# louissmit/VBNN

Hardware: AMD Instinct MI355X
Metric: VBLinear fwd+bwd samples/sec (higher is better)
Workload: dtype bf16; 1 GPU; 784-4096-4096-10 VBLinear MLP, batch 4096 per GPU, LRT, S=1; mode=lrt, global_batch=4096, parallelism=dp1, warmup_steps_run=250, backward_order=every updateGradInput, then the accGradParameters from the first layer up, launch=one stream launch per kernel

## Files before the change

vbnn_amd/csrc/elementwise.hip:

```cpp
#include "common.h"

static inline int grid_for(int64_t work_items, int per_block) {
    int64_t b = (work_items + per_block - 1) / per_block;
    if (b < 1) b = 1;
    if (b > 2048) b = 2048;
    return (int)b;
}

template <bool HW>
__global__ __launch_bounds__(256) void k_fill_normal(float* out, int64_t rows, int64_t cols, int64_t ld, uint64_t seed,
                                                     uint32_t stream, uint32_t layer, uint32_t draw, int64_t row0, float scale) {
    const int64_t quads = (cols + 3) >> 2;
    const int64_t total = rows * quads;
    for (int64_t t = (int64_t)blockIdx.x * 256 + threadIdx.x; t < total; t += (int64_t)gridDim.x * 256) {
        const int64_t r = t / quads, q = t - r * quads;
        const vbnn_f32x4 z = HW ? vbnn_normal4_hw(seed, stream, layer, draw, (uint32_t)(row0 + r), (uint32_t)q)
                                : vbnn_normal4(seed, stream, layer, draw, (uint32_t)(row0 + r), (uint32_t)q);
        float* p = out + r * ld + q * 4;
        const int valid = (int)min((int64_t)4, cols - q * 4);
        const bool vec = ((ld & 3) == 0) && (((uintptr_t)out & 15u) == 0);
        store4<float>(p, z.v[0] * scale, z.v[1] * scale, z.v[2] * scale, z.v[3] * scale, valid, vec);
    }
}

// ... 1289 lines not shown
            const int rr = idx >> 4, c4 = (idx & 15) * 4;
            const int64_t r = r0 + rr, c = c0 + c4;
            float a[4] = {0.f, 0.f, 0.f, 0.f}, b[4] = {0.f, 0.f, 0.f, 0.f};
            const int valid = (r < N) ? (int)min((int64_t)4, I - c) : 0;
            if (valid > 0) {
                load4<float>(src + (rpd > 0 ? r % rpd : r) * ld_src + c, a, valid, vec_in);
#pragma unroll
                for (int e = 0; e < 4; ++e) { const float ar = Elt<T>::from(Elt<T>::to(a[e])); b[e] = ar * ar; }
                store4<T>(x_s + r * ld_x + c, a[0], a[1], a[2], a[3], valid, true);
                if (x2_s) store4<T>(x2_s + r * ld_x + c, b[0], b[1], b[2], b[3], valid, true);
            }
#pragma unroll
            for (int e = 0; e < 4; ++e) { ta[rr][c4 + e] = a[e]; tb[rr][c4 + e] = b[e]; }
        }
        if (xT_s) {
            __syncthreads();
#pragma unroll
            for (int k = 0; k < 4; ++k) {
                const int idx = threadIdx.x + 256 * k;
                const int cc = idx >> 4, r4 = (idx & 15) * 4;
                const int64_t c = c0 + cc, r = r0 + r4;
                const int valid = (c < I) ? (int)min((int64_t)4, N - r) : 0;
                if (valid > 0) {
                    store4<T>(xT_s + c * ld_xT + r, ta[r4][cc], ta[r4 + 1][cc], ta[r4 + 2][cc], ta[r4 + 3][cc], valid, vec_t);
                    if (x2T_s)
                        store4<T>(x2T_s + c * ld_xT + r, tb[r4][cc], tb[r4 + 1][cc], tb[r4 + 2][cc], tb[r4 + 3][cc], valid, vec_t);
                }
            }
            __syncthreads();
        }
    }
}

extern "C" int vbnn_pack_input(vbnn_ctx* ctx, int dtype, const float* src, int64_t ld_src, int64_t N, int64_t I, void* x_s,
                               void* x2_s, int64_t ld_x, void* xT_s, void* x2T_s, int64_t ld_xT, int64_t rows_per_draw) {
    VBNN_API_BEGIN
    VBNN_REQUIRE(ctx && src && x_s, "null argument");
    VBNN_REQUIRE(rows_per_draw >= 0, "rows_per_draw");
    VBNN_REQUIRE(N > 0 && I > 0 && ld_src >= I && ld_x >= I && ld_x % 4 == 0, "shape");
    VBNN_REQUIRE(!x2T_s || xT_s, "x2T_s needs xT_s");
    VBNN_REQUIRE(!xT_s || ld_xT >= N, "ld_xT");
    const int64_t ntiles = ((N + 63) / 64) * ((I + 63) / 64);
    const int nb = (int)(ntiles < 4096 ? ntiles : 4096);
    if (dtype == VBNN_F32)
        hipLaunchKernelGGL(k_pack_input<float>, dim3(nb), dim3(256), 0, ctx->stream, src, ld_src, N, I, (float*)x_s, (float*)x2_s,
                           ld_x, (float*)xT_s, (float*)x2T_s, ld_xT, rows_per_draw);
    else if (dtype == VBNN_BF16)
        hipLaunchKernelGGL(k_pack_input<bf16_t>, dim3(nb), dim3(256), 0, ctx->stream, src, ld_src, N, I, (bf16_t*)x_s,
                           (bf16_t*)x2_s, ld_x, (bf16_t*)xT_s, (bf16_t*)x2T_s, ld_xT, rows_per_draw);
    else { vbnn_set_error("unsupported dtype %d", dtype); return VBNN_ERR_UNSUPPORTED; }
    return vbnn_check_launch("k_pack_input");
    VBNN_API_END
}

template <bool TO_BF16>
__global__ __launch_bounds__(256) void k_cast_grads(const void* __restrict__ src, void* __restrict__ dst, int64_t n, int vec) {
    const int64_t i0 = ((int64_t)blockIdx.x * 256 + threadIdx.x) * 8;
    if (i0 >= n) return;
    if (vec && i0 + 8 <= n) {
        if constexpr (TO_BF16) {
            const f32x4 a = reinterpret_cast<const f32x4*>(static_cast<const float*>(src) + i0)[0];
            const f32x4 b = reinterpret_cast<const f32x4*>(static_cast<const float*>(src) + i0)[1];
            reinterpret_cast<bf16x8*>(static_cast<bf16_t*>(dst) + i0)[0] =
                bf16x8{(bf16_t)a[0], (bf16_t)a[1], (bf16_t)a[2], (bf16_t)a[3], (bf16_t)b[0], (bf16_t)b[1], (bf16_t)b[2], (bf16_t)b[3]};
        } else {
            const bf16x8 v = reinterpret_cast<const bf16x8*>(static_cast<const bf16_t*>(src) + i0)[0];
            reinterpret_cast<f32x4*>(static_cast<float*>(dst) + i0)[0] = f32x4{(float)v[0], (float)v[1], (float)v[2], (float)v[3]};
            reinterpret_cast<f32x4*>(static_cast<float*>(dst) + i0)[1] = f32x4{(float)v[4], (float)v[5], (float)v[6], (float)v[7]};
        }
    } else {
        for (int64_t i = i0; i < n && i < i0 + 8; ++i) {
            if constexpr (TO_BF16) static_cast<bf16_t*>(dst)[i] = (bf16_t)static_cast<const float*>(src)[i];
            else static_cast<float*>(dst)[i] = (float)static_cast<const bf16_t*>(src)[i];
        }
// ... 67 lines not shown
```

vbnn_amd/csrc/head.hip:

```cpp
#include "common.h"
#include "gemm_v1.h"

constexpr int HEAD_CMAX = 16;
constexpr int HEAD_FW = 8;

template <typename T> struct Vec8;
template <> struct Vec8<bf16_t> {
    typedef bf16x8 raw_t;
    static __device__ __forceinline__ raw_t load_raw(const bf16_t* p) { return *reinterpret_cast<const bf16x8*>(p); }
    static __device__ __forceinline__ void cvt(const raw_t& t, float (&v)[8]) {
#pragma unroll
        for (int e = 0; e < 8; ++e) v[e] = (float)t[e];
    }
    static __device__ __forceinline__ raw_t load_guarded(const bf16_t* p, int valid) {
        raw_t t;
#pragma unroll
        for (int e = 0; e < 8; ++e) t[e] = e < valid ? p[e] : (bf16_t)0.f;
        return t;
    }
    static __device__ __forceinline__ void load(const bf16_t* p, float (&v)[8]) {
        const bf16x8 t = *reinterpret_cast<const bf16x8*>(p);
#pragma unroll
        for (int e = 0; e < 8; ++e) v[e] = (float)t[e];
    }
// ... 33 lines not shown
__device__ __forceinline__ float head_sum_partials(const float* src, int64_t stride, int R) {
    float tot = 0.f;
    int r = 0;
    for (; r + 8 <= R; r += 8) {
        float p[8];
#pragma unroll
        for (int u = 0; u < 8; ++u) p[u] = vbnn_load_wt(src + (int64_t)(r + u) * stride);
#pragma unroll
        for (int u = 0; u < 8; ++u) tot += p[u];
    }
    if (r < R) {
        float p[8];
#pragma unroll
        for (int u = 0; u < 8; ++u) p[u] = (r + u < R) ? vbnn_load_wt(src + (int64_t)(r + u) * stride) : 0.f;
#pragma unroll
        for (int u = 0; u < 8; ++u) if (r + u < R) tot += p[u];
    }
    return tot;
}

__device__ __forceinline__ void head_row_max(const float (&v)[4], int q, float& mx, int& arg) {
    mx = -INFINITY; arg = 0x7fffffff;
#pragma unroll
    for (int j = 0; j < 4; ++j)
        if (v[j] > mx) { mx = v[j]; arg = 4 * q + j; }
#pragma unroll
    for (int off = 16; off <= 32; off <<= 1) {
        const float om = __shfl_xor(mx, off, 64);
        const int oa = __shfl_xor(arg, off, 64);
        if (om > mx || (om == mx && oa < arg)) { mx = om; arg = oa; }
    }
}

__device__ __forceinline__ void head_log_softmax(f32x4 s, int q, int C, const float* __restrict__ bias, float (&lg)[4], int& arg, float& lse) {
#pragma unroll
    for (int j = 0; j < 4; ++j) {
        const int c = 4 * q + j;
        lg[j] = (c < C) ? s[j] + (bias ? bias[c] : 0.f) : -INFINITY;
    }
    float mx;
    head_row_max(lg, q, mx, arg);
    float se = 0.f;
#pragma unroll
    for (int j = 0; j < 4; ++j) if (4 * q + j < C) se += expf(lg[j] - mx);
    se += __shfl_xor(se, 16, 64);
    se += __shfl_xor(se, 32, 64);
    lse = mx + logf(se);
}

__device__ __forceinline__ void head_rows_from_logits(f32x4 s, int lane, int64_t n0, int64_t N, int C, const float* __restrict__ bias,
                                                      const int32_t* __restrict__ target, int64_t rpd, float inv_n, float* out, float* g_logits,
                                                      float* logits, double* part_loss, int32_t* part_corr) {
    const int q = lane >> 4, c16 = lane & 15;
    const int64_t n = n0 + c16;
    const bool row_ok = n < N;
    float lg[4];
    int arg;
    float lse;
    head_log_softmax(s, q, C, bias, lg, arg, lse);
    const int t = row_ok ? min(max(target[rpd > 0 ? n % rpd : n], 0), C - 1) : 0;
    double loss_acc = 0.0;
#pragma unroll
    for (int j = 0; j < 4; ++j) {
        const int c = 4 * q + j;
        if (row_ok && c < C) {
            const float o = lg[j] - lse;
            if (logits) logits[n * C + c] = lg[j];
            if (out) out[n * C + c] = o;
            g_logits[n * C + c] = (expf(o) - (c == t ? 1.0f : 0.0f)) * inv_n;
            if (c == t) loss_acc -= (double)o * (double)inv_n;
        }
    }
    int corr = (row_ok && q == 0 && arg == t) ? 1 : 0;
#pragma unroll
    for (int off = 32; off > 0; off >>= 1) { loss_acc += __shfl_xor(loss_acc, off, 64); corr += __shfl_xor(corr, off, 64); }
    if (lane == 0) { vbnn_store_wt(&part_loss[blockIdx.x], loss_acc); vbnn_store_wt(&part_corr[blockIdx.x], (int32_t)corr); }
}

template <int NT>
__device__ __forceinline__ void head_sum_loss_partials(unsigned* counter, const double* part_loss, const int32_t* part_corr, double* loss_sum,
                                                       int32_t* correct, int accumulate, double* red_l, int* red_c, int* last) {
    if (!vbnn_last_arriver(counter, gridDim.x, last)) return;
    const int lane = threadIdx.x & 63, wave = threadIdx.x >> 6;
    double ls = 0.0;
    int cs = 0;
    for (int b = (int)threadIdx.x; b < (int)gridDim.x; b += NT) { ls += vbnn_load_wt(&part_loss[b]); cs += vbnn_load_wt(&part_corr[b]); }
#pragma unroll
    for (int off = 32; off > 0; off >>= 1) { ls += __shfl_xor(ls, off, 64); cs += __shfl_xor(cs, off, 64); }
    if (lane == 0) { red_l[wave] = ls; red_c[wave] = cs; }
    __syncthreads();
    if (threadIdx.x == 0) {
        double lt = 0.0;
        int ct = 0;
#pragma unroll
        for (int w = 0; w < NT / 64; ++w) { lt += red_l[w]; ct += red_c[w]; }
        if (loss_sum) loss_sum[0] = (accumulate ? loss_sum[0] : 0.0) + lt;
        if (correct) correct[0] = (accumulate ? correct[0] : 0) + ct;
    }
}

template <typename T>
__device__ __forceinline__ f32x4 head_logits_wave(const T* __restrict__ hp, const T* __restrict__ wp, int64_t k_lo, int64_t k_hi) {
    constexpr int KE = 64 / (int)sizeof(T);
    typedef typename Frag<T>::type frag_t;
    f32x4 acc = {0.f, 0.f, 0.f, 0.f};
    int64_t ks = k_lo;
    for (; ks + 16 <= k_hi; ks += 16) {
        frag_t a[16], b[16];
#pragma unroll
        for (int u = 0; u < 16; ++u) {
            a[u] = *reinterpret_cast<const frag_t*>(wp + (ks + u) * KE);
            b[u] = *reinterpret_cast<const frag_t*>(hp + (ks + u) * KE);
        }
#pragma unroll
        for (int u = 0; u < 16; ++u) acc = mfma_step<T>(a[u], b[u], acc);
    }
    for (; ks + 8 <= k_hi; ks += 8) {
        frag_t a[8], b[8];
#pragma unroll
// ... 35 lines not shown
    __shared__ int red_c[HEAD_FW];
    __shared__ int last;
    const int lane = threadIdx.x & 63, wave = threadIdx.x >> 6;
    const int64_t n0 = (int64_t)blockIdx.x * 16;
    const int q = lane >> 4, c16 = lane & 15;
    const T* hp = h + min(n0 + c16, N - 1) * ld_h + q * CE;
    const T* wp = w3 + (int64_t)min(c16, C - 1) * ld_w + q * CE;
    const int64_t ksteps = Hp / KE;
    const int64_t k_lo = ksteps * wave / HEAD_FW, k_hi = ksteps * (wave + 1) / HEAD_FW;
    const f32x4 acc = head_logits_wave<T>(hp, wp, k_lo, k_hi);
    part[wave][lane] = acc;
    __syncthreads();
    if (wave == 0) {
        f32x4 s = part[0][lane];
#pragma unroll
        for (int w = 1; w < HEAD_FW; ++w) s += part[w][lane];
        head_rows_from_logits(s, lane, n0, N, C, bias, target, rpd, inv_n, out, g_logits, logits, part_loss, part_corr);
    }
    head_sum_loss_partials<64 * HEAD_FW>(counter, part_loss, part_corr, loss_sum, correct, accumulate, red_l, red_c, &last);
}

__global__ __launch_bounds__(64) void k_head_from_slots(const float* __restrict__ slots, int n_slots, const float* __restrict__ bias,
                                                        const int32_t* __restrict__ target, int64_t N, int C, float inv_n, float* out,
                                                        float* g_logits, float* logits, double* loss_sum, int32_t* correct, int accumulate,
                                                        double* part_loss, int32_t* part_corr, unsigned* counter, int64_t rpd) {
    __shared__ double red_l[1];
    __shared__ int red_c[1];
    __shared__ int last;
    const int lane = threadIdx.x;
    const int64_t n0 = (int64_t)blockIdx.x * 16;
    const int q = lane >> 4, c16 = lane & 15;
    const float* p = slots + (min(n0 + c16, N - 1) * 16 + 4 * q);
    const int64_t stride = N * 16;
    f32x4 s = {0.f, 0.f, 0.f, 0.f};
    int k = 0;
    for (; k + 16 <= n_slots; k += 16) {
        f32x4 v[16];
#pragma unroll
        for (int u = 0; u < 16; ++u) v[u] = *reinterpret_cast<const f32x4*>(p + (int64_t)(k + u) * stride);
#pragma unroll
        for (int u = 0; u < 16; ++u) s += v[u];
    }
    for (; k + 2 <= n_slots; k += 2) {
        f32x4 v[2];
#pragma unroll
        for (int u = 0; u < 2; ++u) v[u] = *reinterpret_cast<const f32x4*>(p + (int64_t)(k + u) * stride);
        s += v[0]; s += v[1];
    }
    for (; k < n_slots; ++k) s += *reinterpret_cast<const f32x4*>(p + (int64_t)k * stride);
    head_rows_from_logits(s, lane, n0, N, C, bias, target, rpd, inv_n, out, g_logits, logits, part_loss, part_corr);
    head_sum_loss_partials<64>(counter, part_loss, part_corr, loss_sum, correct, accumulate, red_l, red_c, &last);
}

__device__ __forceinline__ float head_row_entropy(const float (&o)[4], int q, int C) {
    float e = 0.f;
#pragma unroll
    for (int j = 0; j < 4; ++j) if (4 * q + j < C) e = fmaf(expf(o[j]), o[j], e);
    e += __shfl_xor(e, 16, 64);
    e += __shfl_xor(e, 32, 64);
    return -e;
}

__device__ __forceinline__ float head_logaddexp(float a, float b) {
    const float m = fmaxf(a, b);
    return m + log1pf(expf(fminf(a, b) - m));
}

template <typename T>
__global__ __launch_bounds__(64 * HEAD_FW) void k_head_predict(const T* __restrict__ h, int64_t ld_h, const T* __restrict__ w3, int64_t ld_w,
                                                               const float* __restrict__ bias, const int32_t* __restrict__ target, int64_t R,
                                                               int64_t Hp, int C, int draws, int S, int first, int final_, float* state,
                                                               float* probs, float* log_probs, float* entropy, float* expected_entropy,
                                                               float* mutual_info, int32_t* pred, double* totals, double* part,
                                                               unsigned* counter) {
    constexpr int KE = 64 / (int)sizeof(T);
    constexpr int CE = 16 / (int)sizeof(T);
    __shared__ f32x4 lp_part[2][HEAD_FW][64];
    __shared__ double red[4][HEAD_FW];
    __shared__ int last;
    const int lane = threadIdx.x & 63, wave = threadIdx.x >> 6;
    const int64_t n0 = (int64_t)blockIdx.x * 16;
    const int q = lane >> 4, c16 = lane & 15;
    const int64_t r = n0 + c16;
// ... 343 lines not shown
            for (int rg = 0; rg < 16; ++rg) tot += red[rg * 16 + tid];
            put(&partial_b[(int64_t)blockIdx.y * C + tid], tot);
        }
    }
    if (!fin_tickets) return;
    __shared__ int fin_last;
    if (!vbnn_last_arriver(fin_tickets + blockIdx.x, gridDim.y, &fin_last)) return;
    const int R = (int)gridDim.y;
    const int64_t nw = (int64_t)C * H;
    for (int k = tid; k < C * 64 + 64; k += 256) {
        const bool is_w = k < C * 64;
        const int64_t i = c0 + (is_w ? k & 63 : k - C * 64);
        if (i >= H) continue;
        float* dst = is_w ? (fin_gw ? fin_gw + (int64_t)(k >> 6) * H + i : nullptr) : (fin_gbp ? fin_gbp + i : nullptr);
        if (!dst) continue;
        const float* src = is_w ? partial_w + (int64_t)(k >> 6) * H + i : partial_bp + i;
        const int64_t stride = is_w ? nw : H;
        const float tot = head_sum_partials(src, stride, R);
        *dst = (fin_accumulate ? *dst : 0.f) + tot;
    }
    if (blockIdx.x == 0 && tid < C && fin_gb) {
        const float tot = head_sum_partials(partial_b + tid, C, R);
        fin_gb[tid] = (fin_accumulate ? fin_gb[tid] : 0.f) + tot;
    }
}

typedef __bf16 hb_bf16x2 __attribute__((ext_vector_type(2)));
__device__ __forceinline__ float hb_dot2(unsigned a, unsigned b, float c) {
    return __builtin_amdgcn_fdot2_f32_bf16(__builtin_bit_cast(hb_bf16x2, a), __builtin_bit_cast(hb_bf16x2, b), c, false);
}
__device__ __forceinline__ unsigned hb_bf16_bits(float v) {
    return (unsigned)__builtin_bit_cast(unsigned short, (bf16_t)v);
}
template <int U, int HEAD_SW >
__global__ __launch_bounds__(64 * HEAD_SW) void k_head_backward_stream(
    const bf16_t* __restrict__ h, int64_t ld_h, const bf16_t* __restrict__ w3, int64_t ld_w, const float* __restrict__ g, int64_t N,
    int64_t H, int C, int relu_mask, const bf16_t* __restrict__ r_prev, int64_t ld_r, bf16_t* __restrict__ g_prev,
    bf16_t* __restrict__ gv_prev, int64_t ld_gp, int rows_per_chunk, float* __restrict__ partial_w ,
    float* __restrict__ partial_b , float* __restrict__ partial_bp ,
    unsigned* fin_tickets , int fin_accumulate, float* fin_gw, float* fin_gb, float* fin_gbp) {
    static_assert(U == 2 || U == 4, "2 or 4 hidden units per lane");
    constexpr int CP = 12, NP = CP / 2, UW = U / 2;
    typedef float accv __attribute__((ext_vector_type(U)));
    typedef unsigned rawv __attribute__((ext_vector_type(UW)));
    __shared__ accv red[4][HEAD_SW][64];
    const int tid = threadIdx.x, lane = tid & 63, wave = tid >> 6;
    const int64_t cb0 = (int64_t)blockIdx.x * (64 * U);
    const int64_t c0 = cb0 + U * lane;
    const int64_t n_lo = (int64_t)blockIdx.y * rows_per_chunk, n_hi = min(N, n_lo + rows_per_chunk);
    unsigned wp[NP][U];
    {
        unsigned wr[CP][UW];
#pragma unroll
        for (int c = 0; c < CP; ++c) {
            rawv t = 0u;
            if (c < C) t = *reinterpret_cast<const rawv*>(w3 + (int64_t)c * ld_w + c0);
#pragma unroll
            for (int k = 0; k < UW; ++k) wr[c][k] = ((const unsigned*)&t)[k];
        }
#pragma unroll
        for (int p = 0; p < NP; ++p)
#pragma unroll
            for (int e = 0; e < U; ++e) {
                const unsigned lo = (wr[2 * p][e >> 1] >> (16 * (e & 1))) & 0xffffu, hi = (wr[2 * p + 1][e >> 1] >> (16 * (e & 1))) & 0xffffu;
                wp[p][e] = lo | (hi << 16);
            }
    }
    float accw[CP][U], accb[U], accg = 0.f;
#pragma unroll
    for (int e = 0; e < U; ++e) accb[e] = 0.f;
#pragma unroll
    for (int c = 0; c < CP; ++c)
#pragma unroll
        for (int e = 0; e < U; ++e) accw[c][e] = 0.f;
    const int gcls = lane < CP ? lane : lane - CP;
    const bool gl_on = lane < 2 * CP && gcls < C;
    const bool has_r = r_prev != nullptr;
    const unsigned lo_h = (unsigned)(U * lane);
    auto ldrow = [&](int64_t n, rawv& hv, rawv& rv) {
        hv = *reinterpret_cast<const rawv*>(h + (n * ld_h + cb0) + lo_h);
        rv = 0u;
        if (has_r) rv = *reinterpret_cast<const rawv*>(r_prev + (n * ld_r + cb0) + lo_h);
    };
    auto ldg = [&](int64_t n) { return gl_on ? g[(n + (lane >= CP ? 1 : 0)) * C + gcls] : 0.f; };
    auto word = [](const rawv& v, int k) { return ((const unsigned*)&v)[k]; };
    int64_t n = n_lo + 2 * wave;
    rawv h0 = 0u, h1 = 0u, r0 = 0u, r1 = 0u;
    float gv = 0.f;
    if (n < n_hi) { ldrow(n, h0, r0); ldrow(n + 1, h1, r1); gv = ldg(n); }
    for (; n < n_hi; n += 2 * HEAD_SW) {
        const rawv hh[2] = {h0, h1}, rr[2] = {r0, r1};
        const float cg = gv;
        const int64_t nn = n + 2 * HEAD_SW;
        if (nn < n_hi) { ldrow(nn, h0, r0); ldrow(nn + 1, h1, r1); gv = ldg(nn); }
        accg += cg;
        const unsigned gb = hb_bf16_bits(cg);
        unsigned g0[CP], g1[CP];
#pragma unroll
        for (int c = 0; c < CP; ++c) { g0[c] = __builtin_amdgcn_readlane(gb, c); g1[c] = __builtin_amdgcn_readlane(gb, CP + c); }
#pragma unroll
        for (int row = 0; row < 2; ++row) {
            const unsigned* gs = row ? g1 : g0;
            float gx[U];
#pragma unroll
            for (int e = 0; e < U; ++e) gx[e] = 0.f;
#pragma unroll
            for (int p = 0; p < NP; ++p) {
                const unsigned gp2 = gs[2 * p] | (gs[2 * p + 1] << 16);
#pragma unroll
                for (int e = 0; e < U; ++e) gx[e] = hb_dot2(gp2, wp[p][e], gx[e]);
            }
            unsigned gbits[U], vbits[U];
#pragma unroll
            for (int e = 0; e < U; ++e) {
                const unsigned hw = word(hh[row], e >> 1), rw = word(rr[row], e >> 1);
                const float hv = __builtin_bit_cast(float, (e & 1) ? (hw & 0xffff0000u) : (hw << 16));
                const float rv = __builtin_bit_cast(float, (e & 1) ? (rw & 0xffff0000u) : (rw << 16));
                const float gp = (relu_mask && !(hv > 0.f)) ? 0.f : gx[e];
                gbits[e] = hb_bf16_bits(gp);
                vbits[e] = hb_bf16_bits(has_r ? gp * rv : 0.f);
                accb[e] += __builtin_bit_cast(float, gbits[e] << 16);
            }
            const int64_t ro = (n + row) * ld_gp + cb0;
            rawv og, ov;
#pragma unroll
            for (int k = 0; k < UW; ++k) { ((unsigned*)&og)[k] = gbits[2 * k] | (gbits[2 * k + 1] << 16); ((unsigned*)&ov)[k] = vbits[2 * k] | (vbits[2 * k + 1] << 16); }
            *reinterpret_cast<rawv*>(g_prev + ro + lo_h) = og;
            if (gv_prev) *reinterpret_cast<rawv*>(gv_prev + ro + lo_h) = ov;
        }
        unsigned hp[U];
#pragma unroll
        for (int e = 0; e < U; ++e) {
            const unsigned a = word(hh[0], e >> 1), b = word(hh[1], e >> 1);
            hp[e] = (e & 1) ? ((a >> 16) | (b & 0xffff0000u)) : ((a & 0xffffu) | (b << 16));
        }
#pragma unroll
        for (int c = 0; c < CP; ++c) {
            const unsigned gr2 = g0[c] | (g1[c] << 16);
#pragma unroll
            for (int e = 0; e < U; ++e) accw[c][e] = hb_dot2(gr2, hp[e], accw[c][e]);
        }
    }
    const int64_t chunk = blockIdx.y;
    auto put = [&](float* p, const accv& t) {
        if (!fin_tickets) { *reinterpret_cast<accv*>(p) = t; return; }
#pragma unroll
        for (int e = 0; e < U; e += 2) vbnn_store_wt2(p + e, t[e], t[e + 1]);
    };
    auto meet = [&](const accv (&q)[4], int nq, auto&& emit) {
        __syncthreads();
#pragma unroll
        for (int k = 0; k < 4; ++k)
            if (k < nq) red[k][wave][lane] = q[k];
        __syncthreads();
        if (wave < nq) {
            accv t = red[wave][0][lane];
#pragma unroll
            for (int w = 1; w < HEAD_SW; ++w) t += red[wave][w][lane];
            emit(wave, t);
        }
    };
#pragma unroll
    for (int c4 = 0; c4 < CP; c4 += 4) {
        accv q[4];
#pragma unroll
        for (int k = 0; k < 4; ++k)
#pragma unroll
            for (int e = 0; e < U; ++e) q[k][e] = accw[c4 + k][e];
        meet(q, 4, [&](int k, accv t) {
            if (partial_w && c4 + k < C) put(partial_w + ((chunk * C + c4 + k) * H + c0), t);
        });
    }
    {
        accv q[4];
// ... 357 lines not shown
    if (!sums && !g_prev && !gT_prev) return VBNN_OK;
    static const bool env_read = [] { const char* e = getenv("VBNN_HEAD_INLINE_FINISH"); if (e && e[0] == '0') g_head_inline_finish = 0; return true; }();
    (void)env_read;
    const int64_t tiles_c = (H + 63) / 64, tiles_r = (N + 63) / 64;
    const int64_t per_chunk = C * H + C + H;
    const int64_t cap = (int64_t)(ctx->scratch_doubles * 2) / per_chunk;
    VBNN_REQUIRE(!sums || cap >= 1, "hidden size too large for the reduction scratch");
    int64_t R = (2 * (int64_t)vbnn_cu_count() + tiles_c - 1) / tiles_c;
    static const int env_blocks = [] { const char* e = getenv("VBNN_HEAD_BLOCKS"); return e ? atoi(e) : 0; }();
    if (env_blocks > 0) R = (env_blocks + tiles_c - 1) / tiles_c;
    if (R > tiles_r) R = tiles_r;
    if (sums && R > cap) R = cap;
    if (R < 1) R = 1;
    VBNN_REQUIRE(R <= 65535, "too many row chunks");
    const int rows_per_chunk = (int)((tiles_r + R - 1) / R) * 64;
    R = (N + rows_per_chunk - 1) / rows_per_chunk;
    float* partial_w = reinterpret_cast<float*>(ctx->scratch);
    float* partial_b = partial_w + R * C * H;
    float* partial_bp = partial_b + R * C;
    const bool vec = (ld_h % 8 == 0) && (!r_prev_any || ld_r_prev % 8 == 0) && (!g_prev || ld_gp % 8 == 0) &&
                     (!(gT_prev || gvT_prev) || ld_gpT % 8 == 0) &&
                     ((((uintptr_t)h | (uintptr_t)r_prev_any | (uintptr_t)g_prev | (uintptr_t)gv_prev | (uintptr_t)gT_prev |
                        (uintptr_t)gvT_prev) & 15u) == 0);
    const dim3 grid((unsigned)tiles_c, (unsigned)R);
    float* pw = (gradWeight || gradBias_prev) ? partial_w : nullptr;
    float* pb = gradBias ? partial_b : nullptr;
    float* pbp = gradBias_prev ? partial_bp : nullptr;
    const bool full = vec && (H % 64 == 0) && (N % 64 == 0) && N * ld_h < (1ll << 31) && N * ld_gp < (1ll << 31) &&
                      H * ld_gpT < (1ll << 31) && (!r_prev_any || N * ld_r_prev < (1ll << 31));
    const bool inline_fin = sums && tiles_c * R <= vbnn_cu_count() && tiles_c <= VBNN_CNT_TILES_MAX && g_head_inline_finish;
    unsigned* ft = inline_fin ? ctx->counters + VBNN_CNT_TILES : nullptr;
    static const bool env_stream = [] { const char* e = getenv("VBNN_HEAD_STREAM"); return !(e && e[0] == '0'); }();
    if constexpr (sizeof(T) == 2) {
        const bool want = g_head_stream == 1 || (g_head_stream == -1 && env_stream && !inline_fin);
        if (want && full && C <= 12 && !r_prev && g_prev && !gT_prev && !gvT_prev && H % 128 == 0 && N % 32 == 0) {
            constexpr int SU = 2, SWV = 16;
            if (H % (64 * SU) == 0 && N % (2 * SWV) == 0) {
            const int64_t cb = H / (64 * SU);
            int64_t Rs = ((int64_t)vbnn_cu_count() + cb - 1) / cb;
            if (Rs < 1) Rs = 1;
            if (sums && Rs > cap) Rs = cap;
            const int rpc = (int)(((N + Rs - 1) / Rs + 2 * SWV - 1) / (2 * SWV) * (2 * SWV));
            Rs = (N + rpc - 1) / rpc;
            float* spw = reinterpret_cast<float*>(ctx->scratch);
            float* spb = spw + Rs * C * H;
            float* spbp = spb + Rs * C;
#define VBNN_HS_LAUNCH(UU, WW) hipLaunchKernelGGL((k_head_backward_stream<UU, WW>), dim3((unsigned)cb, (unsigned)Rs), dim3(64 * WW), 0, ctx->stream, (const bf16_t*)h, ld_h, \
                               (const bf16_t*)w3, ld_w, g_logits, N, H, (int)C, relu_mask, (const bf16_t*)r_prev_t, ld_r_prev, (bf16_t*)g_prev,  \
                               (bf16_t*)gv_prev, ld_gp, rpc, (gradWeight || gradBias_prev) ? spw : nullptr, gradBias ? spb : nullptr,         \
                               gradBias_prev ? spbp : nullptr, sft, accumulate, gradWeight, gradBias, gradBias_prev)
            unsigned* sft = (sums && g_head_inline_finish && cb <= VBNN_CNT_TILES_MAX) ? ctx->counters + VBNN_CNT_TILES : nullptr;
            VBNN_HS_LAUNCH(SU, SWV);
#undef VBNN_HS_LAUNCH
            if (sums && !sft) {
                const int64_t outs = C * H + (gradBias_prev ? H : 0);
                hipLaunchKernelGGL(k_head_backward_finish, dim3((unsigned)((outs + 255) / 256)), dim3(256), 0, ctx->stream, spw, spb, spbp,
                                   (int)Rs, H, (int)C, accumulate, gradWeight, gradBias, gradBias_prev);
            }
            return vbnn_check_launch("k_head_backward_stream");
            }
        }
    }
    if (full && C <= 12 && !r_prev)
        hipLaunchKernelGGL((k_head_backward<T, true, true, 12>), grid, dim3(256), 0, ctx->stream, h, ld_h, w3, ld_w, g_logits, N, H, (int)C,
                           relu_mask, r_prev, r_prev_t, ld_r_prev, g_prev, gv_prev, ld_gp, gT_prev, gvT_prev, ld_gpT, rows_per_chunk,
                           pw, pb, pbp, ft, accumulate, gradWeight, gradBias, gradBias_prev);
    else if (full)
        hipLaunchKernelGGL((k_head_backward<T, true, true>), grid, dim3(256), 0, ctx->stream, h, ld_h, w3, ld_w, g_logits, N, H, (int)C,
                           relu_mask, r_prev, r_prev_t, ld_r_prev, g_prev, gv_prev, ld_gp, gT_prev, gvT_prev, ld_gpT, rows_per_chunk,
                           pw, pb, pbp, ft, accumulate, gradWeight, gradBias, gradBias_prev);
    else if (vec)
        hipLaunchKernelGGL((k_head_backward<T, true, false>), grid, dim3(256), 0, ctx->stream, h, ld_h, w3, ld_w, g_logits, N, H, (int)C,
                           relu_mask, r_prev, r_prev_t, ld_r_prev, g_prev, gv_prev, ld_gp, gT_prev, gvT_prev, ld_gpT, rows_per_chunk,
                           pw, pb, pbp, ft, accumulate, gradWeight, gradBias, gradBias_prev);
    else
        hipLaunchKernelGGL((k_head_backward<T, false, false>), grid, dim3(256), 0, ctx->stream, h, ld_h, w3, ld_w, g_logits, N, H, (int)C,
                           relu_mask, r_prev, r_prev_t, ld_r_prev, g_prev, gv_prev, ld_gp, gT_prev, gvT_prev, ld_gpT, rows_per_chunk,
                           pw, pb, pbp, ft, accumulate, gradWeight, gradBias, gradBias_prev);
    if (sums && !inline_fin) {
        const int64_t outs = C * H + (gradBias_prev ? H : 0);
        hipLaunchKernelGGL(k_head_backward_finish, dim3((unsigned)((outs + 255) / 256)), dim3(256), 0, ctx->stream, partial_w,
                           partial_b, partial_bp, (int)R, H, (int)C, accumulate, gradWeight, gradBias, gradBias_prev);
    }
    return vbnn_check_launch("k_head_backward");
}
// ... 73 lines not shown
```

Measured before the change: 5.333 million samples/s.

## Add row-wise input pack kernel and DPP-widened head backward stream accesses

Adds a row-major pack kernel for the input, used when no transposed copy is needed. It converts 8 floats per thread to bf16 along with their squares, using vector loads and stores, in place of the 64x64 tile-transpose kernel. The head backward stream kernel gains an access-width template: the default AW=2 has lane pairs load and store 8-byte words across two rows and swaps halves with DPP, and an optional AW=4 uses a quad transpose. The head forward reduction hoists the bias and target loads ahead of the slot sums, unrolls the slot sum to 32, and unrolls the partial-loss sum by 4. These changes aim to widen global memory transactions in bandwidth-bound small kernels, at the cost of extra cross-lane shuffles and more register use.

```diff
diff --git a/vbnn_amd/csrc/elementwise.hip b/vbnn_amd/csrc/elementwise.hip
--- a/vbnn_amd/csrc/elementwise.hip
+++ b/vbnn_amd/csrc/elementwise.hip
@@ -1345,6 +1345,81 @@
     }
 }
 
+constexpr int PACK_U = 2;
+template <typename T>
+__global__ __launch_bounds__(256) void k_pack_input_rows(const float* __restrict__ src, int64_t ld_src, int64_t I, T* __restrict__ x_s,
+                                                         T* __restrict__ x2_s, int64_t ld_x, int64_t rpd, int64_t pieces_per_row,
+                                                         int64_t npieces, int vec_in, int vec_out) {
+    const int64_t g0 = (int64_t)blockIdx.x * (256 * PACK_U) + threadIdx.x;
+    float v[PACK_U][8];
+    int valid[PACK_U];
+    int64_t off[PACK_U];
+#pragma unroll
+    for (int u = 0; u < PACK_U; ++u) {
+        const int64_t g = g0 + 256 * u;
+        valid[u] = 0;
+        off[u] = 0;
+#pragma unroll
+        for (int e = 0; e < 8; ++e) v[u][e] = 0.f;
+        if (g < npieces) {
+            const int64_t r = g / pieces_per_row, c = (g - r * pieces_per_row) * 8;
+            valid[u] = (int)min((int64_t)8, I - c);
+            off[u] = r * ld_x + c;
+            const float* sp = src + (rpd > 0 ? r % rpd : r) * ld_src + c;
+            if (vec_in && valid[u] == 8) {
+                const f32x4 lo = *reinterpret_cast<const f32x4*>(sp), hi = *reinterpret_cast<const f32x4*>(sp + 4);
+#pragma unroll
+                for (int e = 0; e < 4; ++e) { v[u][e] = lo[e]; v[u][4 + e] = hi[e]; }
+            } else {
+#pragma unroll
+                for (int e = 0; e < 8; ++e) if (e < valid[u]) v[u][e] = sp[e];
+            }
+        }
+    }
+#pragma unroll
+    for (int u = 0; u < PACK_U; ++u) {
+        if (valid[u] == 0) continue;
+        T a[8], b[8];
+#pragma unroll
+        for (int e = 0; e < 8; ++e) {
+            a[e] = Elt<T>::to(v[u][e]);
+            const float ar = Elt<T>::from(a[e]);
+            b[e] = Elt<T>::to(ar * ar);
+        }
+        if (vec_out && valid[u] == 8) {
+            constexpr int Q = 16 / (int)sizeof(T);
+            typedef T vecq __attribute__((ext_vector_type(Q)));
+#pragma unroll
+            for (int k = 0; k < 8 / Q; ++k) {
+                vecq ta, tb;
+#pragma unroll
+                for (int e = 0; e < Q; ++e) { ta[e] = a[k * Q + e]; tb[e] = b[k * Q + e]; }
+                *reinterpret_cast<vecq*>(x_s + off[u] + k * Q) = ta;
+                if (x2_s) *reinterpret_cast<vecq*>(x2_s + off[u] + k * Q) = tb;
+            }
+        } else {
+#pragma unroll
+            for (int e = 0; e < 8; ++e)
+                if (e < valid[u]) {
+                    x_s[off[u] + e] = a[e];
+                    if (x2_s) x2_s[off[u] + e] = b[e];
+                }
+        }
+    }
+}
+
+template <typename T>
+static void pack_input_rows(vbnn_ctx* ctx, const float* src, int64_t ld_src, int64_t N, int64_t I, T* x_s, T* x2_s, int64_t ld_x,
+                            int64_t rpd) {
+    const int64_t ppr = (I + 7) / 8, npieces = N * ppr;
+    constexpr int64_t Q = 16 / (int64_t)sizeof(T);
+    const int vec_in = (ld_src % 4 == 0) && (((uintptr_t)src & 15u) == 0);
+    const int vec_out = (ld_x % Q == 0) && ((((uintptr_t)x_s | (uintptr_t)x2_s) & 15u) == 0);
+    const int64_t per_block = 256 * PACK_U;
+    hipLaunchKernelGGL(k_pack_input_rows<T>, dim3((unsigned)((npieces + per_block - 1) / per_block)), dim3(256), 0, ctx->stream, src,
+                       ld_src, I, x_s, x2_s, ld_x, rpd, ppr, npieces, vec_in, vec_out);
+}
+
 extern "C" int vbnn_pack_input(vbnn_ctx* ctx, int dtype, const float* src, int64_t ld_src, int64_t N, int64_t I, void* x_s,
                                void* x2_s, int64_t ld_x, void* xT_s, void* x2T_s, int64_t ld_xT, int64_t rows_per_draw) {
     VBNN_API_BEGIN
@@ -1353,6 +1428,13 @@
     VBNN_REQUIRE(N > 0 && I > 0 && ld_src >= I && ld_x >= I && ld_x % 4 == 0, "shape");
     VBNN_REQUIRE(!x2T_s || xT_s, "x2T_s needs xT_s");
     VBNN_REQUIRE(!xT_s || ld_xT >= N, "ld_xT");
+    static const bool env_rows = [] { const char* e = getenv("VBNN_PACK_ROWS"); return !(e && e[0] == '0'); }();
+    if (!xT_s && env_rows && N * ((I + 7) / 8) < (1ll << 40)) {
+        if (dtype == VBNN_F32) pack_input_rows<float>(ctx, src, ld_src, N, I, (float*)x_s, (float*)x2_s, ld_x, rows_per_draw);
+        else if (dtype == VBNN_BF16) pack_input_rows<bf16_t>(ctx, src, ld_src, N, I, (bf16_t*)x_s, (bf16_t*)x2_s, ld_x, rows_per_draw);
+        else { vbnn_set_error("unsupported dtype %d", dtype); return VBNN_ERR_UNSUPPORTED; }
+        return vbnn_check_launch("k_pack_input_rows");
+    }
     const int64_t ntiles = ((N + 63) / 64) * ((I + 63) / 64);
     const int nb = (int)(ntiles < 4096 ? ntiles : 4096);
     if (dtype == VBNN_F32)
diff --git a/vbnn_amd/csrc/head.hip b/vbnn_amd/csrc/head.hip
--- a/vbnn_amd/csrc/head.hip
+++ b/vbnn_amd/csrc/head.hip
@@ -89,11 +89,15 @@
     }
 }
 
-__device__ __forceinline__ void head_log_softmax(f32x4 s, int q, int C, const float* __restrict__ bias, float (&lg)[4], int& arg, float& lse) {
+__device__ __forceinline__ void head_load_bias(const float* __restrict__ bias, int q, int C, float (&bv)[4]) {
+#pragma unroll
+    for (int j = 0; j < 4; ++j) bv[j] = (bias && 4 * q + j < C) ? bias[4 * q + j] : 0.f;
+}
+__device__ __forceinline__ void head_log_softmax_v(f32x4 s, int q, int C, const float (&bv)[4], float (&lg)[4], int& arg, float& lse) {
 #pragma unroll
     for (int j = 0; j < 4; ++j) {
         const int c = 4 * q + j;
-        lg[j] = (c < C) ? s[j] + (bias ? bias[c] : 0.f) : -INFINITY;
+        lg[j] = (c < C) ? s[j] + bv[j] : -INFINITY;
     }
     float mx;
     head_row_max(lg, q, mx, arg);
@@ -104,18 +108,25 @@
     se += __shfl_xor(se, 32, 64);
     lse = mx + logf(se);
 }
-
-__device__ __forceinline__ void head_rows_from_logits(f32x4 s, int lane, int64_t n0, int64_t N, int C, const float* __restrict__ bias,
-                                                      const int32_t* __restrict__ target, int64_t rpd, float inv_n, float* out, float* g_logits,
-                                                      float* logits, double* part_loss, int32_t* part_corr) {
+__device__ __forceinline__ void head_log_softmax(f32x4 s, int q, int C, const float* __restrict__ bias, float (&lg)[4], int& arg, float& lse) {
+    float bv[4];
+    head_load_bias(bias, q, C, bv);
+    head_log_softmax_v(s, q, C, bv, lg, arg, lse);
+}
+
+__device__ __forceinline__ int head_load_target(const int32_t* __restrict__ target, int64_t n, int64_t N, int64_t rpd, int C) {
+    return n < N ? min(max(target[rpd > 0 ? n % rpd : n], 0), C - 1) : 0;
+}
+__device__ __forceinline__ void head_rows_from_logits_v(f32x4 s, int lane, int64_t n0, int64_t N, int C, const float (&bv)[4], int t,
+                                                        float inv_n, float* out, float* g_logits, float* logits, double* part_loss,
+                                                        int32_t* part_corr) {
     const int q = lane >> 4, c16 = lane & 15;
     const int64_t n = n0 + c16;
     const bool row_ok = n < N;
     float lg[4];
     int arg;
     float lse;
-    head_log_softmax(s, q, C, bias, lg, arg, lse);
-    const int t = row_ok ? min(max(target[rpd > 0 ? n % rpd : n], 0), C - 1) : 0;
+    head_log_softmax_v(s, q, C, bv, lg, arg, lse);
     double loss_acc = 0.0;
 #pragma unroll
     for (int j = 0; j < 4; ++j) {
@@ -133,6 +144,14 @@
     for (int off = 32; off > 0; off >>= 1) { loss_acc += __shfl_xor(loss_acc, off, 64); corr += __shfl_xor(corr, off, 64); }
     if (lane == 0) { vbnn_store_wt(&part_loss[blockIdx.x], loss_acc); vbnn_store_wt(&part_corr[blockIdx.x], (int32_t)corr); }
 }
+__device__ __forceinline__ void head_rows_from_logits(f32x4 s, int lane, int64_t n0, int64_t N, int C, const float* __restrict__ bias,
+                                                      const int32_t* __restrict__ target, int64_t rpd, float inv_n, float* out, float* g_logits,
+                                                      float* logits, double* part_loss, int32_t* part_corr) {
+    float bv[4];
+    head_load_bias(bias, lane >> 4, C, bv);
+    const int t = head_load_target(target, n0 + (lane & 15), N, rpd, C);
+    head_rows_from_logits_v(s, lane, n0, N, C, bv, t, inv_n, out, g_logits, logits, part_loss, part_corr);
+}
 
 template <int NT>
 __device__ __forceinline__ void head_sum_loss_partials(unsigned* counter, const double* part_loss, const int32_t* part_corr, double* loss_sum,
@@ -141,7 +160,18 @@
     const int lane = threadIdx.x & 63, wave = threadIdx.x >> 6;
     double ls = 0.0;
     int cs = 0;
-    for (int b = (int)threadIdx.x; b < (int)gridDim.x; b += NT) { ls += vbnn_load_wt(&part_loss[b]); cs += vbnn_load_wt(&part_corr[b]); }
+    const int nb = (int)gridDim.x;
+    int b = (int)threadIdx.x;
+    for (; b < nb; b += 4 * NT) {
+        double pl[4] = {0.0, 0.0, 0.0, 0.0};
+        int pc[4] = {0, 0, 0, 0};
+#pragma unroll
+        for (int u = 0; u < 4; ++u)
+            if (b + u * NT < nb) { pl[u] = vbnn_load_wt(&part_loss[b + u * NT]); pc[u] = vbnn_load_wt(&part_corr[b + u * NT]); }
+#pragma unroll
+        for (int u = 0; u < 4; ++u)
+            if (b + u * NT < nb) { ls += pl[u]; cs += pc[u]; }
+    }
 #pragma unroll
     for (int off = 32; off > 0; off >>= 1) { ls += __shfl_xor(ls, off, 64); cs += __shfl_xor(cs, off, 64); }
     if (lane == 0) { red_l[wave] = ls; red_c[wave] = cs; }
@@ -243,8 +273,18 @@
     const int q = lane >> 4, c16 = lane & 15;
     const float* p = slots + (min(n0 + c16, N - 1) * 16 + 4 * q);
     const int64_t stride = N * 16;
+    float bv[4];
+    head_load_bias(bias, q, C, bv);
+    const int t = head_load_target(target, n0 + c16, N, rpd, C);
     f32x4 s = {0.f, 0.f, 0.f, 0.f};
     int k = 0;
+    for (; k + 32 <= n_slots; k += 32) {
+        f32x4 v[32];
+#pragma unroll
+        for (int u = 0; u < 32; ++u) v[u] = *reinterpret_cast<const f32x4*>(p + (int64_t)(k + u) * stride);
+#pragma unroll
+        for (int u = 0; u < 32; ++u) s += v[u];
+    }
     for (; k + 16 <= n_slots; k += 16) {
         f32x4 v[16];
 #pragma unroll
@@ -259,7 +299,7 @@
         s += v[0]; s += v[1];
     }
     for (; k < n_slots; ++k) s += *reinterpret_cast<const f32x4*>(p + (int64_t)k * stride);
-    head_rows_from_logits(s, lane, n0, N, C, bias, target, rpd, inv_n, out, g_logits, logits, part_loss, part_corr);
+    head_rows_from_logits_v(s, lane, n0, N, C, bv, t, inv_n, out, g_logits, logits, part_loss, part_corr);
     head_sum_loss_partials<64>(counter, part_loss, part_corr, loss_sum, correct, accumulate, red_l, red_c, &last);
 }
 
@@ -669,7 +709,28 @@
 __device__ __forceinline__ unsigned hb_bf16_bits(float v) {
     return (unsigned)__builtin_bit_cast(unsigned short, (bf16_t)v);
 }
-template <int U, int HEAD_SW >
+template <int AW>
+__device__ __forceinline__ void hb_pair_swap(unsigned& a , unsigned& b , bool odd) {
+    if constexpr (AW == 2) {
+        const unsigned send = odd ? a : b;
+        const unsigned recv = (unsigned)__builtin_amdgcn_update_dpp(0, (int)send, 0xB1, 0xF, 0xF, false);
+        a = odd ? recv : a;
+        b = odd ? b : recv;
+    }
+}
+__device__ __forceinline__ void hb_quad_transpose(unsigned (&w)[4], int j) {
+    const bool b0 = (j & 1) != 0, b1 = (j & 2) != 0;
+    auto net = [&](unsigned (&x)[4]) {
+        const unsigned a = b0 ? x[1] : x[0], b = b0 ? x[0] : x[1], c = b0 ? x[3] : x[2], d = b0 ? x[2] : x[3];
+        x[0] = b1 ? c : a; x[1] = b1 ? d : b; x[2] = b1 ? a : c; x[3] = b1 ? b : d;
+    };
+    net(w);
+    w[1] = (unsigned)__builtin_amdgcn_update_dpp(0, (int)w[1], 0xB1, 0xF, 0xF, false);
+    w[2] = (unsigned)__builtin_amdgcn_update_dpp(0, (int)w[2], 0x4E, 0xF, 0xF, false);
+    w[3] = (unsigned)__builtin_amdgcn_update_dpp(0, (int)w[3], 0x1B, 0xF, 0xF, false);
+    net(w);
+}
+template <int U, int HEAD_SW , int AW = 1>
 __global__ __launch_bounds__(64 * HEAD_SW) void k_head_backward_stream(
     const bf16_t* __restrict__ h, int64_t ld_h, const bf16_t* __restrict__ w3, int64_t ld_w, const float* __restrict__ g, int64_t N,
     int64_t H, int C, int relu_mask, const bf16_t* __restrict__ r_prev, int64_t ld_r, bf16_t* __restrict__ g_prev,
@@ -677,6 +738,7 @@
     float* __restrict__ partial_b , float* __restrict__ partial_bp ,
     unsigned* fin_tickets , int fin_accumulate, float* fin_gw, float* fin_gb, float* fin_gbp) {
     static_assert(U == 2 || U == 4, "2 or 4 hidden units per lane");
+    static_assert(AW == 1 || ((AW == 2 || AW == 4) && U == 2), "the exchanges move one owned word per lane and row");
     constexpr int CP = 12, NP = CP / 2, UW = U / 2;
     typedef float accv __attribute__((ext_vector_type(U)));
     typedef unsigned rawv __attribute__((ext_vector_type(UW)));
@@ -719,17 +781,22 @@
         rv = 0u;
         if (has_r) rv = *reinterpret_cast<const rawv*>(r_prev + (n * ld_r + cb0) + lo_h);
     };
+    const bool odd = (lane & 1) != 0;
+    const unsigned lo_p = (unsigned)(4 * (lane >> 1));
+    auto ldpair = [&](int64_t n, rawv& ha, rawv& hb, rawv& ra, rawv& rb) {
+        if constexpr (AW == 2) {
+            const int64_t nr = n + (odd ? 1 : 0);
+            const uint2 th = *reinterpret_cast<const uint2*>(h + (nr * ld_h + cb0) + lo_p);
+            uint2 tr = {0u, 0u};
+            if (has_r) tr = *reinterpret_cast<const uint2*>(r_prev + (nr * ld_r + cb0) + lo_p);
+            ha = th.x; hb = th.y; ra = tr.x; rb = tr.y;
+        } else {
+            ldrow(n, ha, ra); ldrow(n + 1, hb, rb);
+        }
+    };
     auto ldg = [&](int64_t n) { return gl_on ? g[(n + (lane >= CP ? 1 : 0)) * C + gcls] : 0.f; };
     auto word = [](const rawv& v, int k) { return ((const unsigned*)&v)[k]; };
-    int64_t n = n_lo + 2 * wave;
-    rawv h0 = 0u, h1 = 0u, r0 = 0u, r1 = 0u;
-    float gv = 0.f;
-    if (n < n_hi) { ldrow(n, h0, r0); ldrow(n + 1, h1, r1); gv = ldg(n); }
-    for (; n < n_hi; n += 2 * HEAD_SW) {
-        const rawv hh[2] = {h0, h1}, rr[2] = {r0, r1};
-        const float cg = gv;
-        const int64_t nn = n + 2 * HEAD_SW;
-        if (nn < n_hi) { ldrow(nn, h0, r0); ldrow(nn + 1, h1, r1); gv = ldg(nn); }
+    auto pair = [&](int64_t n, const rawv (&hh)[2], const rawv (&rr)[2], float cg, rawv (&ogs)[2], rawv (&ovs)[2]) {
         accg += cg;
         const unsigned gb = hb_bf16_bits(cg);
         unsigned g0[CP], g1[CP];
@@ -762,8 +829,11 @@
             rawv og, ov;
 #pragma unroll
             for (int k = 0; k < UW; ++k) { ((unsigned*)&og)[k] = gbits[2 * k] | (gbits[2 * k + 1] << 16); ((unsigned*)&ov)[k] = vbits[2 * k] | (vbits[2 * k + 1] << 16); }
-            *reinterpret_cast<rawv*>(g_prev + ro + lo_h) = og;
-            if (gv_prev) *reinterpret_cast<rawv*>(gv_prev + ro + lo_h) = ov;
+            ogs[row] = og; ovs[row] = ov;
+            if constexpr (AW == 1) {
+                *reinterpret_cast<rawv*>(g_prev + ro + lo_h) = og;
+                if (gv_prev) *reinterpret_cast<rawv*>(gv_prev + ro + lo_h) = ov;
+            }
         }
         unsigned hp[U];
 #pragma unroll
@@ -777,6 +847,76 @@
 #pragma unroll
             for (int e = 0; e < U; ++e) accw[c][e] = hb_dot2(gr2, hp[e], accw[c][e]);
         }
+    };
+    int64_t n = n_lo + 2 * wave;
+    if constexpr (AW == 4) {
+        const int j = lane & 3;
+        const unsigned lo_q = (unsigned)(8 * (lane >> 2));
+        auto qrow = [&](int64_t n, bool two) { return n + (j & 1) + ((two && j >= 2) ? 2 * HEAD_SW : 0); };
+        auto ldquad = [&](int64_t n, uint4& hq, uint4& rq) {
+            const int64_t nr = qrow(n, n + 2 * HEAD_SW < n_hi);
+            hq = *reinterpret_cast<const uint4*>(h + (nr * ld_h + cb0) + lo_q);
+            rq = uint4{0u, 0u, 0u, 0u};
+            if (has_r) rq = *reinterpret_cast<const uint4*>(r_prev + (nr * ld_r + cb0) + lo_q);
+        };
+        uint4 hq = {0u, 0u, 0u, 0u}, rq = {0u, 0u, 0u, 0u};
+        float gva = 0.f, gvb = 0.f;
+        if (n < n_hi) { ldquad(n, hq, rq); gva = ldg(n); if (n + 2 * HEAD_SW < n_hi) gvb = ldg(n + 2 * HEAD_SW); }
+        for (; n < n_hi; n += 4 * HEAD_SW) {
+            const bool two = n + 2 * HEAD_SW < n_hi;
+            unsigned hw[4] = {hq.x, hq.y, hq.z, hq.w}, rw[4] = {rq.x, rq.y, rq.z, rq.w};
+            const float cga = gva, cgb = gvb;
+            const int64_t nn = n + 4 * HEAD_SW;
+            if (nn < n_hi) { ldquad(nn, hq, rq); gva = ldg(nn); if (nn + 2 * HEAD_SW < n_hi) gvb = ldg(nn + 2 * HEAD_SW); }
+            hb_quad_transpose(hw, j);
+            if (has_r) hb_quad_transpose(rw, j);
+            unsigned ow[4] = {0u, 0u, 0u, 0u}, vw[4] = {0u, 0u, 0u, 0u};
+            {
+                const rawv hh[2] = {hw[0], hw[1]}, rr[2] = {rw[0], rw[1]};
+                rawv ogs[2], ovs[2];
+                pair(n, hh, rr, cga, ogs, ovs);
+                ow[0] = word(ogs[0], 0); ow[1] = word(ogs[1], 0); vw[0] = word(ovs[0], 0); vw[1] = word(ovs[1], 0);
+            }
+            if (two) {
+                const rawv hh[2] = {hw[2], hw[3]}, rr[2] = {rw[2], rw[3]};
+                rawv ogs[2], ovs[2];
+                pair(n + 2 * HEAD_SW, hh, rr, cgb, ogs, ovs);
+                ow[2] = word(ogs[0], 0); ow[3] = word(ogs[1], 0); vw[2] = word(ovs[0], 0); vw[3] = word(ovs[1], 0);
+            }
+            const int64_t ro = qrow(n, two) * ld_gp + cb0;
+            const bool st = two || j < 2;
+            hb_quad_transpose(ow, j);
+            if (st) *reinterpret_cast<uint4*>(g_prev + ro + lo_q) = uint4{ow[0], ow[1], ow[2], ow[3]};
+            if (gv_prev) {
+                hb_quad_transpose(vw, j);
+                if (st) *reinterpret_cast<uint4*>(gv_prev + ro + lo_q) = uint4{vw[0], vw[1], vw[2], vw[3]};
+            }
+        }
+    } else {
+    rawv h0 = 0u, h1 = 0u, r0 = 0u, r1 = 0u;
+    float gv = 0.f;
+    if (n < n_hi) { ldpair(n, h0, h1, r0, r1); gv = ldg(n); }
+    for (; n < n_hi; n += 2 * HEAD_SW) {
+        rawv hh[2] = {h0, h1}, rr[2] = {r0, r1};
+        const float cg = gv;
+        const int64_t nn = n + 2 * HEAD_SW;
+        if (nn < n_hi) { ldpair(nn, h0, h1, r0, r1); gv = ldg(nn); }
+        if constexpr (AW == 2) {
+            hb_pair_swap<AW>(((unsigned*)&hh[0])[0], ((unsigned*)&hh[1])[0], odd);
+            if (has_r) hb_pair_swap<AW>(((unsigned*)&rr[0])[0], ((unsigned*)&rr[1])[0], odd);
+        }
+        rawv ogs[2], ovs[2];
+        pair(n, hh, rr, cg, ogs, ovs);
+        if constexpr (AW == 2) {
+            const int64_t ro = (n + (odd ? 1 : 0)) * ld_gp + cb0;
+            hb_pair_swap<AW>(((unsigned*)&ogs[0])[0], ((unsigned*)&ogs[1])[0], odd);
+            *reinterpret_cast<uint2*>(g_prev + ro + lo_p) = uint2{word(ogs[0], 0), word(ogs[1], 0)};
+            if (gv_prev) {
+                hb_pair_swap<AW>(((unsigned*)&ovs[0])[0], ((unsigned*)&ovs[1])[0], odd);
+                *reinterpret_cast<uint2*>(gv_prev + ro + lo_p) = uint2{word(ovs[0], 0), word(ovs[1], 0)};
+            }
+        }
+    }
     }
     const int64_t chunk = blockIdx.y;
     auto put = [&](float* p, const accv& t) {
@@ -1200,8 +1340,10 @@
     unsigned* ft = inline_fin ? ctx->counters + VBNN_CNT_TILES : nullptr;
     static const bool env_stream = [] { const char* e = getenv("VBNN_HEAD_STREAM"); return !(e && e[0] == '0'); }();
     if constexpr (sizeof(T) == 2) {
-        const bool want = g_head_stream == 1 || (g_head_stream == -1 && env_stream && !inline_fin);
-        if (want && full && C <= 12 && !r_prev && g_prev && !gT_prev && !gvT_prev && H % 128 == 0 && N % 32 == 0) {
+        const bool fits = vec && H % 128 == 0 && N % 32 == 0 && N * ld_h < (1ll << 31) && N * ld_gp < (1ll << 31) &&
+                          (!r_prev_any || N * ld_r_prev < (1ll << 31));
+        const bool want = (g_head_stream == 1 && fits) || (g_head_stream == -1 && env_stream && !inline_fin && full);
+        if (want && C <= 12 && !r_prev && g_prev && !gT_prev && !gvT_prev && H % 128 == 0 && N % 32 == 0) {
             constexpr int SU = 2, SWV = 16;
             if (H % (64 * SU) == 0 && N % (2 * SWV) == 0) {
             const int64_t cb = H / (64 * SU);
@@ -1213,12 +1355,14 @@
             float* spw = reinterpret_cast<float*>(ctx->scratch);
             float* spb = spw + Rs * C * H;
             float* spbp = spb + Rs * C;
-#define VBNN_HS_LAUNCH(UU, WW) hipLaunchKernelGGL((k_head_backward_stream<UU, WW>), dim3((unsigned)cb, (unsigned)Rs), dim3(64 * WW), 0, ctx->stream, (const bf16_t*)h, ld_h, \
+#define VBNN_HS_LAUNCH(UU, WW, AA) hipLaunchKernelGGL((k_head_backward_stream<UU, WW, AA>), dim3((unsigned)cb, (unsigned)Rs), dim3(64 * WW), 0, ctx->stream, (const bf16_t*)h, ld_h, \
                                (const bf16_t*)w3, ld_w, g_logits, N, H, (int)C, relu_mask, (const bf16_t*)r_prev_t, ld_r_prev, (bf16_t*)g_prev,  \
                                (bf16_t*)gv_prev, ld_gp, rpc, (gradWeight || gradBias_prev) ? spw : nullptr, gradBias ? spb : nullptr,         \
                                gradBias_prev ? spbp : nullptr, sft, accumulate, gradWeight, gradBias, gradBias_prev)
             unsigned* sft = (sums && g_head_inline_finish && cb <= VBNN_CNT_TILES_MAX) ? ctx->counters + VBNN_CNT_TILES : nullptr;
-            VBNN_HS_LAUNCH(SU, SWV);
+            static const bool env_aw1 = [] { const char* e = getenv("VBNN_HEAD_STREAM_AW"); return e && e[0] == '1'; }();
+            static const bool env_aw4 = [] { const char* e = getenv("VBNN_HEAD_STREAM_AW"); return e && e[0] == '4'; }();
+            if (env_aw1) VBNN_HS_LAUNCH(SU, SWV, 1); else if (env_aw4) VBNN_HS_LAUNCH(SU, SWV, 4); else VBNN_HS_LAUNCH(SU, SWV, 2);
 #undef VBNN_HS_LAUNCH
             if (sums && !sft) {
                 const int64_t outs = C * H + (gradBias_prev ? H : 0);
```

Result: no change. 5.321 million samples/s (-0.2%).
